# DelphinusLab/halo2-gpu-specific

Hardware: AMD Instinct MI355X
Metric: NTT Fr-ops/s @ k=24 (forward+inverse 2^24 BN254 Fr NTT; MSM G1-adds/s under 'msm') (higher is better)
Workload: dtype u32x8 (254-bit Montgomery, integer)

## Files before the change

halo2-gpu-specific_amd/csrc/field.hpp:

```cpp
#pragma once
#ifdef __HIPCC_RTC__
typedef unsigned char uint8_t;
typedef unsigned short uint16_t;
typedef unsigned int uint32_t;
typedef unsigned long uint64_t;
typedef int int32_t;
typedef long int64_t;
#else
#include <hip/hip_runtime.h>
#include <stdint.h>
#endif

namespace h2 {

struct FrParams {
    static constexpr uint32_t MOD[8] = {0xf0000001u, 0x43e1f593u, 0x79b97091u, 0x2833e848u,
                                        0x8181585du, 0xb85045b6u, 0xe131a029u, 0x30644e72u};
    static constexpr uint32_t MOD2[8] = {0xe0000002u, 0x87c3eb27u, 0xf372e122u, 0x5067d090u,
                                         0x0302b0bau, 0x70a08b6du, 0xc2634053u, 0x60c89ce5u};
    static constexpr uint32_t MOD4[8] = {0xc0000004u, 0x0f87d64fu, 0xe6e5c245u, 0xa0cfa121u,
                                         0x06056174u, 0xe14116dau, 0x84c680a6u, 0xc19139cbu};
    static constexpr uint32_t NMOD[8] = {0x0fffffffu, 0xbc1e0a6cu, 0x86468f6eu, 0xd7cc17b7u,
                                         0x7e7ea7a2u, 0x47afba49u, 0x1ece5fd6u, 0xcf9bb18du};
    static constexpr uint32_t PINV256[8] = {0xefffffffu, 0xc2e1f593u, 0x4c6911b3u, 0x6586864bu,
// ... 348 lines not shown
    d.l[1] = subb_co(a.l[1], b.l[1], ca);
    u.l[0] = add_co(d.l[0], P::MOD2[0], cb);
#pragma unroll
    for (int i = 2; i < 8; i++) {
        d.l[i] = subb_co(a.l[i], b.l[i], ca);
        u.l[i - 1] = addc_co(d.l[i - 1], P::MOD2[i - 1], cb);
    }
    u.l[7] = addc_co(d.l[7], P::MOD2[7], cb);
#pragma unroll
    for (int i = 0; i < 8; i++) r.l[i] = sel_co(d.l[i], u.l[i], ca);
    return r;
#else
    return fp_lazy_red2p(fp_lazy_sub(a, b));
#endif
}
template <class P>
H2_DEV Fp<P> fp_lazy_canon(const Fp<P>& a) {
    return fp_reduce_once(fp_lazy_red2p(a));
}

template <int CL>
struct alignas(16) FpChunk {
    uint32_t w[64 / CL];
};

H2_DEV void mad_acc(uint64_t& lo, uint32_t& hi, uint32_t a, uint32_t b) {
#if defined(H2_PORTABLE_MUL) || !defined(__HIP_DEVICE_COMPILE__)
    uint64_t p = (uint64_t)a * b;
    uint64_t s = lo + p;
    hi += (s < p) ? 1u : 0u;
    lo = s;
#else
    uint64_t carry;
    asm("v_mad_u64_u32 %0, %1, %2, %3, %0" : "+v"(lo), "=s"(carry) : "v"(a), "v"(b));
    asm("v_addc_co_u32 %0, %1, %0, 0, %1" : "+v"(hi), "+s"(carry));
#endif
}

template <class P>
__device__ __forceinline__ Fp<P> fp_mul_dev(const Fp<P>& a, const Fp<P>& b);
template <class P>
__device__ __forceinline__ Fp<P> fp_sqr_dev(const Fp<P>& a);
template <class P>
__device__ __forceinline__ Fp<P> fp_mul2_dev(const Fp<P>& a, const Fp<P>& b, const Fp<P>& c, const Fp<P>& d);
template <class P>
__device__ __forceinline__ Fp<P> fp_mul_wide_dev(const Fp<P>& a, const Fp<P>& b);
template <class P>
__device__ __forceinline__ Fp<P> fp_mul_const_dev(const Fp<P>& a, const Fp<P>& w, const Fp<P>& wq);
template <class P, int CL>
__device__ __forceinline__ Fp<P> fp_mul_chunk_dev(const Fp<P>& a, const FpChunk<CL>& t);
#if defined(__HIP_DEVICE_COMPILE__) && !defined(H2_PORTABLE_MUL)
#include "fp_mul_gen.hpp"
#endif

template <class P>
H2_DEV Fp<P> fp_mul(const Fp<P>& a, const Fp<P>& b) {
#if !defined(__HIP_DEVICE_COMPILE__)
    {
        typedef unsigned __int128 u128;
        uint64_t x[4], y[4], p[4];
        for (int i = 0; i < 4; i++) {
            x[i] = (uint64_t)a.l[2 * i] | ((uint64_t)a.l[2 * i + 1] << 32);
            y[i] = (uint64_t)b.l[2 * i] | ((uint64_t)b.l[2 * i + 1] << 32);
            p[i] = (uint64_t)P::MOD[2 * i] | ((uint64_t)P::MOD[2 * i + 1] << 32);
        }
        uint64_t inv = p[0];
        for (int i = 0; i < 6; i++) inv *= 2 - p[0] * inv;
        inv = 0 - inv;
        uint64_t t[6] = {0, 0, 0, 0, 0, 0};
        for (int i = 0; i < 4; i++) {
            u128 c = 0;
            for (int j = 0; j < 4; j++) {
                c += (u128)t[j] + (u128)x[j] * y[i];
                t[j] = (uint64_t)c;
                c >>= 64;
            }
            c += t[4];
            t[4] = (uint64_t)c;
            t[5] = (uint64_t)(c >> 64);
            const uint64_t m = t[0] * inv;
            c = ((u128)t[0] + (u128)m * p[0]) >> 64;
            for (int j = 1; j < 4; j++) {
                c += (u128)t[j] + (u128)m * p[j];
                t[j - 1] = (uint64_t)c;
                c >>= 64;
            }
            c += t[4];
            t[3] = (uint64_t)c;
            t[4] = t[5] + (uint64_t)(c >> 64);
        }
        Fp<P> r;
        for (int i = 0; i < 4; i++) {
            r.l[2 * i] = (uint32_t)t[i];
            r.l[2 * i + 1] = (uint32_t)(t[i] >> 32);
        }
        return fp_reduce_once(r);
    }
#elif !defined(H2_PORTABLE_MUL)
    return fp_mul_dev(a, b);
#endif
    Fp<P> r;
    uint64_t lo = 0;
    uint32_t hi = 0;
    uint32_t m[8];
#pragma unroll
    for (int i = 0; i < 8; i++) {
#pragma unroll
        for (int j = 0; j <= i; j++) mad_acc(lo, hi, a.l[j], b.l[i - j]);
#pragma unroll
        for (int j = 0; j < i; j++) mad_acc(lo, hi, m[j], P::MOD[i - j]);
        m[i] = (uint32_t)lo * P::INV;
        mad_acc(lo, hi, m[i], P::MOD[0]);
        lo = (lo >> 32) | ((uint64_t)hi << 32);
        hi = 0;
    }
#pragma unroll
    for (int i = 8; i < 16; i++) {
#pragma unroll
        for (int j = i - 7; j < 8; j++) mad_acc(lo, hi, a.l[j], b.l[i - j]);
#pragma unroll
        for (int j = i - 7; j < 8; j++) mad_acc(lo, hi, m[j], P::MOD[i - j]);
        r.l[i - 8] = (uint32_t)lo;
        lo = (lo >> 32) | ((uint64_t)hi << 32);
        hi = 0;
    }
    return fp_reduce_once(r);
}

template <class P>
H2_DEV Fp<P> fp_sqr(const Fp<P>& a) {
#if defined(__HIP_DEVICE_COMPILE__) && !defined(H2_PORTABLE_MUL) && !defined(H2_NO_SQR)
    return fp_sqr_dev(a);
#else
    return fp_mul(a, a);
#endif
}

template <class P>
H2_DEV Fp<P> fp_mul2(const Fp<P>& a, const Fp<P>& b, const Fp<P>& c, const Fp<P>& d) {
#if defined(__HIP_DEVICE_COMPILE__) && !defined(H2_PORTABLE_MUL) && !defined(H2_NO_MUL2)
    return fp_mul2_dev(a, b, c, d);
#else
    return fp_add(fp_mul(a, b), fp_mul(c, d));
#endif
}

template <class P>
H2_DEV Fp<P> fp_mul_wide(const Fp<P>& a, const Fp<P>& b) {
#if defined(__HIP_DEVICE_COMPILE__) && !defined(H2_PORTABLE_MUL)
    return fp_mul_wide_dev(a, b);
#else
    Fp<P> r;
    uint64_t lo = 0;
    uint32_t hi = 0;
    uint32_t m[8];
    for (int i = 0; i < 8; i++) {
        for (int j = 0; j <= i; j++) mad_acc(lo, hi, a.l[j], b.l[i - j]);
        for (int j = 0; j < i; j++) mad_acc(lo, hi, m[j], P::MOD[i - j]);
        m[i] = (uint32_t)lo * P::INV;
        mad_acc(lo, hi, m[i], P::MOD[0]);
        lo = (lo >> 32) | ((uint64_t)hi << 32);
        hi = 0;
    }
    for (int i = 8; i < 16; i++) {
        for (int j = i - 7; j < 8; j++) mad_acc(lo, hi, a.l[j], b.l[i - j]);
        for (int j = i - 7; j < 8; j++) mad_acc(lo, hi, m[j], P::MOD[i - j]);
        r.l[i - 8] = (uint32_t)lo;
        lo = (lo >> 32) | ((uint64_t)hi << 32);
        hi = 0;
    }
    return r;
#endif
}

template <class P>
H2_DEV Fp<P> fp_mul_const(const Fp<P>& x, const Fp<P>& w, const Fp<P>& wq) {
#if defined(__HIP_DEVICE_COMPILE__) && !defined(H2_PORTABLE_MUL)
    Fp<P> r = fp_mul_const_dev(x, w, wq);
    if (__builtin_expect(r.l[7] >= P::MOD2[7], 0)) r = fp_lazy_red2p(r);
    return r;
#else
    uint32_t q[8];
    {
        uint64_t lo = 0;
        uint32_t hi = 0;
        for (int i = 0; i < 15; i++) {
            for (int j = (i > 7 ? i - 7 : 0); j <= (i < 7 ? i : 7); j++) mad_acc(lo, hi, x.l[j], wq.l[i - j]);
            if (i >= 8) q[i - 8] = (uint32_t)lo;
            lo = (lo >> 32) | ((uint64_t)hi << 32);
            hi = 0;
        }
        q[7] = (uint32_t)lo;
    }
    Fp<P> r;
    uint64_t lo = 0;
    uint32_t hi = 0;
    for (int i = 0; i < 8; i++) {
        for (int j = 0; j <= i; j++) {
            mad_acc(lo, hi, x.l[j], w.l[i - j]);
            mad_acc(lo, hi, q[j], P::NMOD[i - j]);
        }
        r.l[i] = (uint32_t)lo;
        lo = (lo >> 32) | ((uint64_t)hi << 32);
        hi = 0;
    }
    return r;
#endif
}
template <class P>
H2_DEV void fp_const_pair(const Fp<P>& w_mont, Fp<P>& w_plain, Fp<P>& wq) {
    w_plain = fp_from_mont(w_mont);
    uint64_t lo = 0;
    uint32_t hi = 0;
    for (int i = 0; i < 8; i++) {
        for (int j = 0; j <= i; j++) mad_acc(lo, hi, w_mont.l[j], P::PINV256[i - j]);
        wq.l[i] = (uint32_t)lo;
        lo = (lo >> 32) | ((uint64_t)hi << 32);
        hi = 0;
    }
}

template <int CL, class P>
H2_DEV Fp<P> fp_mul_chunk(const Fp<P>& x, const FpChunk<CL>& t) {
#if defined(__HIP_DEVICE_COMPILE__) && !defined(H2_PORTABLE_MUL)
    return fp_mul_chunk_dev<P, CL>(x, t);
#else
    constexpr int NC = 8 / CL, NM = CL + 1;
    Fp<P> r;
    uint64_t lo = 0;
    uint32_t hi = 0;
    uint32_t m[NM];
    for (int i = 0; i < NM + 7; i++) {
        for (int j = 0; j < 8; j++) {
            const int l = i - j % CL;
            if (l >= 0 && l <= 7) mad_acc(lo, hi, x.l[j], t.w[l * NC + j / CL]);
        }
        for (int j = 0; j < NM && j < i; j++)
            if (i - j <= 7) mad_acc(lo, hi, m[j], P::MOD[i - j]);
        if (i < NM) {
            m[i] = (uint32_t)lo * P::INV;
            mad_acc(lo, hi, m[i], P::MOD[0]);
        } else {
            r.l[i - NM] = (uint32_t)lo;
        }
        lo = (lo >> 32) | ((uint64_t)hi << 32);
        hi = 0;
    }
    r.l[7] = (uint32_t)lo;
    return r;
#endif
}
template <int AH, bool SREG = false, class P, class Fetch>
H2_DEV Fp<P> fp_mul_chunk_planes(const Fp<P>& x, Fetch&& fetch) {
#if defined(__HIP_DEVICE_COMPILE__) && !defined(H2_PORTABLE_MUL)
    if constexpr (SREG) return fp_mul_chunk1_splanes_dev<AH>(x, fetch);
    else return fp_mul_chunk1_planes_dev<AH>(x, fetch);
#else
    FpChunk<1> t;
    for (int c = 0; c < 8; c++) {
        uint32_t w[8];
        fetch(w, c);
        for (int k = 0; k < 8; k++) t.w[8 * c + k] = w[k];
    }
    return fp_mul_chunk<1>(x, t);
#endif
}
enum FirstPair { FIRST_PAIR_2P = 0, FIRST_PAIR_4P = 1, FIRST_PAIR_CANON = 2 };
template <class P, class Mul>
H2_DEV void fp_lazy_first_pair_mul(Fp<P>& x0, Fp<P>& x1, Fp<P>& x2, Fp<P>& x3, Mul&& mul, const FirstPair form) {
    Fp<P> y0, y1, y2;
    if (form == FIRST_PAIR_CANON) {
        y0 = fp_lazy_add(x0, x1);
        y1 = fp_lazy_sub_off<1>(x0, x1);
        y2 = fp_lazy_add(x2, x3);
    } else {
        if (form == FIRST_PAIR_4P) {
            x0 = fp_lazy_red2p(x0);
            x1 = fp_lazy_red2p(x1);
            x2 = fp_lazy_red2p(x2);
            x3 = fp_lazy_red2p(x3);
        }
        y0 = fp_lazy_add_red(x0, x1);
        y1 = fp_lazy_sub_red(x0, x1);
        y2 = fp_lazy_red2p(fp_lazy_add(x2, x3));
    }
    const Fp<P> y3 = mul(fp_lazy_sub(x2, x3));
    x0 = fp_lazy_add(y0, y2);
    x1 = fp_lazy_add(y1, y3);
    x2 = fp_lazy_sub(y0, y2);
    x3 = fp_lazy_sub(y1, y3);
}
template <int CL, class P>
H2_DEV void fp_lazy_first_pair_of(Fp<P>& x0, Fp<P>& x1, Fp<P>& x2, Fp<P>& x3, const FpChunk<CL>& w3, const FirstPair form) {
    fp_lazy_first_pair_mul(x0, x1, x2, x3, [&w3](const Fp<P>& d) { return fp_mul_chunk(d, w3); }, form);
}
template <int CL, class P>
H2_DEV void fp_lazy_first_pair(Fp<P>& x0, Fp<P>& x1, Fp<P>& x2, Fp<P>& x3, const FpChunk<CL>& w3, const bool red) {
    fp_lazy_first_pair_of(x0, x1, x2, x3, w3, red ? FIRST_PAIR_4P : FIRST_PAIR_2P);
}
template <int CL, class P>
H2_DEV void fp_lazy_first_pair_canon(Fp<P>& x0, Fp<P>& x1, Fp<P>& x2, Fp<P>& x3, const FpChunk<CL>& w3) {
    fp_lazy_first_pair_of(x0, x1, x2, x3, w3, FIRST_PAIR_CANON);
}
template <int CL, class P>
H2_DEV void fp_chunk_table(const Fp<P>& w_mont, FpChunk<CL>& out) {
    constexpr int NC = 8 / CL;
    const Fp<P> w_plain = fp_from_mont(w_mont);
    for (int k = 0; k < NC; k++) {
        Fp<P> c;
        for (int l = 0; l < 8; l++) c.l[l] = P::CHUNK_POW[CL * k + CL - 1][l];
        const Fp<P> t = fp_mul(w_plain, c);
        for (int l = 0; l < 8; l++) out.w[l * NC + k] = t.l[l];
    }
}

template <class P>
H2_DEV Fp<P> fp_to_mont(const Fp<P>& canon) {
    Fp<P> rr;
#pragma unroll
    for (int i = 0; i < 8; i++) rr.l[i] = P::RR[i];
    return fp_reduce_once(fp_mul_wide(canon, rr));
}
template <class P>
H2_DEV Fp<P> fp_from_mont(const Fp<P>& a) {
    Fp<P> one = fp_zero<P>();
    one.l[0] = 1;
    return fp_reduce_once(fp_mul_wide(a, one));
}

template <class P>
H2_DEV Fp<P> fp_inv(const Fp<P>& a) {
    uint32_t u[8], v[8], r[8], s[8];
    uint32_t nz = 0;
#pragma unroll
    for (int i = 0; i < 8; i++) {
        u[i] = P::MOD[i];
        v[i] = a.l[i];
        r[i] = 0;
        s[i] = i == 0 ? 1u : 0u;
        nz |= a.l[i];
    }
    if (nz == 0) return a;
    uint32_t k = 0;
    auto halve = [](uint32_t* x) {
#pragma unroll
        for (int i = 0; i < 8; i++) x[i] = (x[i] >> 1) | (i < 7 ? x[i + 1] << 31 : 0u);
    };
    auto dbl = [](uint32_t* x) {
#pragma unroll
        for (int i = 7; i >= 0; i--) x[i] = (x[i] << 1) | (i ? x[i - 1] >> 31 : 0u);
    };
    auto sub = [](uint32_t* x, const uint32_t* y) {
        uint32_t bw = 0;
#pragma unroll
        for (int i = 0; i < 8; i++) {
            const uint32_t d = x[i] - y[i], b1 = x[i] < y[i] ? 1u : 0u, e = d - bw, b2 = d < bw ? 1u : 0u;
            x[i] = e;
            bw = b1 | b2;
        }
    };
    auto add = [](uint32_t* x, const uint32_t* y) {
        uint32_t cy = 0;
#pragma unroll
        for (int i = 0; i < 8; i++) {
            const uint32_t t = x[i] + y[i], c1 = t < y[i] ? 1u : 0u, e = t + cy, c2 = e < cy ? 1u : 0u;
            x[i] = e;
            cy = c1 | c2;
        }
    };
    auto greater = [](const uint32_t* x, const uint32_t* y) {
#pragma unroll
        for (int i = 7; i >= 0; i--)
            if (x[i] != y[i]) return x[i] > y[i];
        return false;
    };
    for (;;) {
        uint32_t vnz = 0;
#pragma unroll
        for (int i = 0; i < 8; i++) vnz |= v[i];
        if (vnz == 0) break;
        if ((u[0] & 1) == 0) {
            halve(u);
            dbl(s);
        } else if ((v[0] & 1) == 0) {
            halve(v);
            dbl(r);
        } else if (greater(u, v)) {
            sub(u, v);
            halve(u);
            add(r, s);
            dbl(s);
        } else {
            sub(v, u);
            halve(v);
            add(s, r);
            dbl(r);
        }
        k++;
    }
    Fp<P> x;
    {
        uint32_t d[8];
        uint64_t bw = 0;
#pragma unroll
        for (int i = 0; i < 8; i++) {
            uint64_t e = (uint64_t)r[i] - P::MOD[i] - bw;
            d[i] = (uint32_t)e;
            bw = (e >> 32) & 1;
        }
        uint64_t bw2 = 0;
#pragma unroll
        for (int i = 0; i < 8; i++) {
            const uint32_t rr = bw ? r[i] : d[i];
            uint64_t e = (uint64_t)P::MOD[i] - rr - bw2;
            x.l[i] = (uint32_t)e;
            bw2 = (e >> 32) & 1;
        }
    }
    x = fp_reduce_once(x);
    for (uint32_t i = k; i < 512; i++) x = fp_dbl(x);
    return x;
}

template <class P>
H2_DEV Fp<P> fp_pow_u32(const Fp<P>& a, uint32_t e) {
    if (e == 0) return fp_one<P>();
    Fp<P> acc = a;
    for (int i = 30 - __builtin_clz(e); i >= 0; i--) {
        acc = fp_sqr(acc);
        if ((e >> i) & 1) acc = fp_mul(acc, a);
    }
    return acc;
}

}
```

halo2-gpu-specific_amd/csrc/ntt_pass.hip:

```cpp
#include <stdexcept>

#include "ntt_pass.hpp"

namespace h2 {

__device__ __forceinline__ void tw_store(Fr* out, uint32_t i, const Fr& w_mont, uint32_t pair) {
    if (!pair) {
        fp_store(out + i, w_mont);
        return;
    }
    if (pair == 2) {
        TwChunk t;
        fp_chunk_table(w_mont, t);
        uint4* const q = reinterpret_cast<uint4*>(out) + (size_t)i * TW_CHUNK_Q;
#pragma unroll
        for (uint32_t k = 0; k < TW_CHUNK_Q; k++) q[k] = make_uint4(t.w[4 * k], t.w[4 * k + 1], t.w[4 * k + 2], t.w[4 * k + 3]);
        return;
    }
    if (pair == 3) {
        TwChunk32 t;
        fp_chunk_table(w_mont, t);
        uint4* const q = reinterpret_cast<uint4*>(out) + (size_t)i * TW_CHUNK32_Q;
#pragma unroll
        for (uint32_t k = 0; k < TW_CHUNK32_Q; k++) q[k] = make_uint4(t.w[4 * k], t.w[4 * k + 1], t.w[4 * k + 2], t.w[4 * k + 3]);
// ... 46 lines not shown
        hi >>= a.prevB[q];
        K |= d << a.prevT[q];
    }
    return K;
}
__device__ __forceinline__ uint32_t K_to_hi(uint32_t K, const PassArgs& a) {
    uint32_t hi = 0;
    for (uint32_t q = 0; q < a.nprev; q++) {
        uint32_t d = (K >> a.prevT[q]) & ((1u << a.prevB[q]) - 1);
        hi = (hi << a.prevB[q]) | d;
    }
    return hi;
}

__device__ __forceinline__ Fr twiddle_pow(const PassArgs& a, uint32_t e) {
    if (a.log_n <= LO_BITS) return fp_load(a.tw_lo + e);
    Fr lo = fp_load(a.tw_lo + (e & ((1u << LO_BITS) - 1)));
    Fr hi = fp_load(a.tw_hi + (e >> LO_BITS));
    return fp_mul(lo, hi);
}

extern __shared__ __attribute__((aligned(16))) uint4 h2_smem[];

__device__ __forceinline__ Fr lds_get(const uint4* lo, const uint4* hi, uint32_t i) {
    uint4 a = lo[i], b = hi[i];
    Fr r;
    r.l[0] = a.x; r.l[1] = a.y; r.l[2] = a.z; r.l[3] = a.w;
    r.l[4] = b.x; r.l[5] = b.y; r.l[6] = b.z; r.l[7] = b.w;
    return r;
}
__device__ __forceinline__ void lds_put(uint4* lo, uint4* hi, uint32_t i, const Fr& v) {
    lo[i] = make_uint4(v.l[0], v.l[1], v.l[2], v.l[3]);
    hi[i] = make_uint4(v.l[4], v.l[5], v.l[6], v.l[7]);
}

__device__ __forceinline__ Fr store_twiddle(const PassArgs& a, const Fr& y, const uint32_t entry) {
    const uint4* const q = reinterpret_cast<const uint4*>(a.nx_tab) + (size_t)entry * TW_CHUNK_Q;
    TwChunk t;
#pragma unroll
    for (uint32_t k = 0; k < TW_CHUNK_Q; k++) {
        const uint4 v = q[k];
        t.w[4 * k] = v.x; t.w[4 * k + 1] = v.y; t.w[4 * k + 2] = v.z; t.w[4 * k + 3] = v.w;
    }
    return fp_mul_chunk(y, t);
}

template <bool RADIX4, bool NLAST = false, bool ST = false>
__global__ void __launch_bounds__(512, 4) k_ntt_pass(PassArgs a) {
    constexpr bool CW = RADIX4;
    static_assert(!ST || NLAST || !RADIX4, "a last pass stores the transform's output");
    const bool is_last = NLAST ? false : a.is_last != 0;
    auto tmul = [](const Fr& x, const Fr& w) -> Fr { return fp_mul_wide(x, w); };
    const uint32_t B = a.B, R = 1u << B, log_c = a.log_c, C = 1u << log_c;
    const uint32_t zskip = a.zskip;
    uint4* t_lo = h2_smem;
    uint4* t_hi = t_lo + (R << log_c);
    uint4* w_lo = t_hi + (R << log_c);
    uint4* w_hi = w_lo + (R >> 1) + (CW ? 0 : 1);
    uint4* q_lo = w_hi + (R >> 1);
    uint4* q_hi = q_lo + (R >> 1);
    struct Tw {
        Fr w, q;
    };
    auto tw_get = [&](uint32_t i) __attribute__((always_inline)) -> Tw {
        Tw t;
        t.w = lds_get(w_lo, w_hi, i);
        if constexpr (CW) t.q = lds_get(q_lo, q_hi, i);
        return t;
    };
    auto bmul = [](const Fr& x, const Tw& t) __attribute__((always_inline)) -> Fr {
        if constexpr (CW) return fp_mul_const(x, t.w, t.q);
        else return fp_mul_wide(x, t.w);
    };
    const uint32_t nthreads = blockDim.x;
    const uint32_t tid = threadIdx.x;
    const Fr* const in_p = a.batch ? a.in_b[blockIdx.y] : a.in;
    Fr* const out_p = a.batch ? a.out_b[blockIdx.y] : a.out;
    const uint32_t n_mask = (a.log_n >= 32) ? 0xffffffffu : ((1u << a.log_n) - 1);

    for (uint32_t i = tid; i < (R >> 1); i += nthreads) {
        if constexpr (CW) {
            lds_put(w_lo, w_hi, i, fp_load(a.tw_bfly + 2 * i));
            lds_put(q_lo, q_hi, i, fp_load(a.tw_bfly + 2 * i + 1));
        } else {
            lds_put(w_lo, w_hi, i, fp_load(a.tw_bfly + i));
        }
    }

    const uint32_t tile_id = blockIdx.x;
    const uint32_t total = R << log_c;

    uint32_t base = 0, K_uniform = 0;
    const uint32_t S = 1u << a.s_log;
    if (!is_last) {
        uint32_t chunks_per_hi = S >> log_c;
        uint32_t hi = tile_id / chunks_per_hi, lo0 = (tile_id % chunks_per_hi) << log_c;
        base = (hi << (B + a.s_log)) + lo0;
        K_uniform = hi_to_K(hi, a);
    }

    constexpr uint32_t NE = RADIX4 ? 4 : 2;
    for (uint32_t e0 = tid; e0 < total; e0 += NE * nthreads) {
        uint32_t rho[NE], col[NE], idx[NE], Kk[NE];
        bool live[NE];
        Fr x[NE];
#pragma unroll
        for (uint32_t q = 0; q < NE; q++) {
            const uint32_t e = e0 + q * nthreads;
            if (!is_last) {
                col[q] = e & (C - 1);
                rho[q] = (e >> log_c) & (R - 1);
                idx[q] = base + (rho[q] << a.s_log) + col[q];
                Kk[q] = K_uniform;
            } else {
                rho[q] = e & (R - 1);
                col[q] = (e >> B) & (C - 1);
                Kk[q] = (tile_id << log_c) + col[q];
                idx[q] = (K_to_hi(Kk[q], a) << B) + rho[q];
            }
            live[q] = e < total && !(zskip && rho[q] >= (R >> zskip));
        }
#pragma unroll
        for (uint32_t q = 0; q < NE; q++) {
            x[q] = fp_zero<FrParams>();
            if (live[q] && idx[q] < a.in_len) x[q] = fp_load(in_p + idx[q]);
        }
        if (a.has_pre3) {
#pragma unroll
            for (uint32_t q = 0; q < NE; q++) {
                const uint32_t m = idx[q] % 3;
                Fr w;
#pragma unroll
                for (int l = 0; l < 8; l++) w.l[l] = m == 1 ? a.pre3[1].l[l] : a.pre3[2].l[l];
                if (m != 0) x[q] = tmul(x[q], w);
            }
        }
        const bool pre_scale = a.scale_mode == 1u && a.nprev == 0;
        if ((a.nprev != 0 && !a.tw_applied) || pre_scale) {
            if (!NLAST && a.tw_direct != nullptr && !pre_scale) {
#pragma unroll
                for (uint32_t q0 = 0; q0 < NE; q0 += 2) {
                    Fr w[2];
#pragma unroll
                    for (uint32_t q = 0; q < 2; q++) w[q] = fp_load(a.tw_direct + ((Kk[q0 + q] << B) | rho[q0 + q]));
#pragma unroll
                    for (uint32_t q = 0; q < 2; q++) x[q0 + q] = tmul(x[q0 + q], w[q]);
                }
            } else if (a.log_n <= LO_BITS && !pre_scale) {
#pragma unroll
                for (uint32_t q = 0; q < NE; q++) {
                    const uint32_t ex = (uint32_t)(((uint64_t)rho[q] * Kk[q]) << a.s_log) & n_mask;
                    x[q] = tmul(x[q], fp_load(a.tw_lo + ex));
                }
            } else {
                const Fr* const two_lo = pre_scale ? a.sc_lo : a.tw_lo;
                const Fr* const two_hi = pre_scale ? a.sc_hi : a.tw_hi;
#pragma unroll
                for (uint32_t q0 = 0; q0 < NE; q0 += 2) {
                    Fr wl[2], wh[2];
#pragma unroll
                    for (uint32_t q = 0; q < 2; q++) {
                        const uint32_t ex = pre_scale ? (idx[q0 + q] & n_mask)
                                                      : ((uint32_t)(((uint64_t)rho[q0 + q] * Kk[q0 + q]) << a.s_log) & n_mask);
                        wl[q] = fp_load(two_lo + (ex & ((1u << LO_BITS) - 1)));
                        wh[q] = fp_load(two_hi + (ex >> LO_BITS));
                    }
#pragma unroll
                    for (uint32_t q = 0; q < 2; q++) x[q0 + q] = tmul(x[q0 + q], fp_mul(wl[q], wh[q]));
                }
            }
        }
#pragma unroll
        for (uint32_t q = 0; q < NE; q++) {
            const uint32_t e = e0 + q * nthreads;
            const uint32_t r_q = is_last ? (e & (R - 1)) : ((e >> log_c) & (R - 1));
            const uint32_t c_q = is_last ? ((e >> B) & (C - 1)) : (e & (C - 1));
            if (e >= total || (zskip && r_q >= (R >> zskip))) continue;
            if (zskip) {
                for (uint32_t m = 0; m < (1u << zskip); m++) lds_put(t_lo, t_hi, ((bitrev(r_q, B) | m) << log_c) + c_q, x[q]);
            } else {
                lds_put(t_lo, t_hi, (bitrev(r_q, B) << log_c) + c_q, x[q]);
            }
        }
    }
    __syncthreads();

    uint32_t s0 = zskip;
    if constexpr (RADIX4) {
        const uint32_t nunits = total >> 2;
        auto round4 = [&](const uint32_t s) __attribute__((always_inline)) {
            const uint32_t h = 1u << s;
            const uint32_t log_per = (B - 2 + log_c) - s;
            const bool by_r = s != 0 && log_per >= 6 && (nthreads & 63) == 0;
            for (uint32_t t = tid; t < nunits; t += nthreads) {
                uint32_t c, r, p;
                if (by_r) {
                    r = t >> log_per;
                    const uint32_t j = t & ((1u << log_per) - 1);
                    c = j & (C - 1);
                    p = ((j >> log_c) << (s + 2)) | r;
                } else {
                    c = t & (C - 1);
                    const uint32_t b = t >> log_c;
                    r = b & (h - 1);
                    p = ((b >> s) << (s + 2)) | r;
                }
                const uint32_t i0 = (p << log_c) + c, step = h << log_c;
                Fr x0 = lds_get(t_lo, t_hi, i0), x1 = lds_get(t_lo, t_hi, i0 + step);
                Fr x2 = lds_get(t_lo, t_hi, i0 + 2 * step), x3 = lds_get(t_lo, t_hi, i0 + 3 * step);
                const bool unit = s == 0 || (by_r && r == 0);
                x0 = fp_lazy_red2p(x0);
                x2 = fp_lazy_red2p(x2);
                if (!unit) {
                    const Tw wa = tw_get(r << (B - 1 - s));
                    x1 = bmul(x1, wa);
                    x3 = bmul(x3, wa);
                } else {
                    x1 = fp_lazy_red2p(x1);
                    x3 = fp_lazy_red2p(x3);
                }
                const Fr y0 = fp_lazy_add_red(x0, x1), y1 = fp_lazy_sub_red(x0, x1);
                Fr y2 = fp_lazy_add(x2, x3), y3 = fp_lazy_sub(x2, x3);
                y2 = unit ? fp_lazy_red2p(y2) : bmul(y2, tw_get(r << (B - 2 - s)));
                y3 = bmul(y3, tw_get((r + h) << (B - 2 - s)));
                lds_put(t_lo, t_hi, i0, fp_lazy_add(y0, y2));
                lds_put(t_lo, t_hi, i0 + 2 * step, fp_lazy_sub(y0, y2));
                lds_put(t_lo, t_hi, i0 + step, fp_lazy_add(y1, y3));
                lds_put(t_lo, t_hi, i0 + 3 * step, fp_lazy_sub(y1, y3));
            }
            __syncthreads();
        };
        for (; s0 + 1 < B; s0 += 2) round4(s0);
    }
    const uint32_t nbf = total >> 1;
    for (uint32_t s = s0; s < B; s++) {
        const uint32_t h = 1u << s;
        const uint32_t log_per = (B - 1 + log_c) - s;
        const bool by_r = s != 0 && log_per >= 6 && (nthreads & 63) == 0;
        for (uint32_t t = tid; t < nbf; t += nthreads) {
            uint32_t c, r, i;
            if (by_r) {
                r = t >> log_per;
                uint32_t j = t & ((1u << log_per) - 1);
                c = j & (C - 1);
                i = ((j >> log_c) << (s + 1)) | r;
            } else {
                c = t & (C - 1);
                uint32_t b = t >> log_c;
                r = b & (h - 1);
                i = ((b >> s) << (s + 1)) | r;
            }
            const uint32_t iu = (i << log_c) + c, iv = ((i + h) << log_c) + c;
            Fr u = lds_get(t_lo, t_hi, iu), v = lds_get(t_lo, t_hi, iv);
            const bool skip = s == 0 || (by_r && r == 0);
            u = fp_lazy_red2p(u);
            v = skip ? fp_lazy_red2p(v) : bmul(v, tw_get(r << (B - 1 - s)));
            lds_put(t_lo, t_hi, iu, fp_lazy_add(u, v));
            lds_put(t_lo, t_hi, iv, fp_lazy_sub(u, v));
        }
        __syncthreads();
    }

    for (uint32_t e0 = tid; e0 < total; e0 += NE * nthreads) {
        Fr y[NE];
        uint32_t idx[NE];
#pragma unroll
        for (uint32_t q = 0; q < NE; q++) {
            const uint32_t e = e0 + q * nthreads;
            const uint32_t c = e & (C - 1), k = (e >> log_c) & (R - 1);
            if (!is_last)
                idx[q] = base + (k << a.s_log) + c;
            else
                idx[q] = ((tile_id << log_c) + c) + (k << a.t_log);
            y[q] = lds_get(t_lo, t_hi, (k << log_c) + c);
        }
        if (is_last && a.scale_mode == 2u) {
#pragma unroll
            for (uint32_t q = 0; q < NE; q++) {
                const uint32_t i = idx[q] & n_mask;
                const Fr w = fp_mul(fp_load(a.sc_lo + (i & ((1u << LO_BITS) - 1))), fp_load(a.sc_hi + (i >> LO_BITS)));
                y[q] = fp_reduce_once(fp_mul_wide(y[q], w));
            }
        } else if (is_last && a.has_post3 && !a.hi_scaled) {
#pragma unroll
            for (uint32_t q = 0; q < NE; q++) {
                const uint32_t m = idx[q] % 3;
                Fr w;
#pragma unroll
                for (int l = 0; l < 8; l++) w.l[l] = m == 0 ? a.post3[0].l[l] : (m == 1 ? a.post3[1].l[l] : a.post3[2].l[l]);
                y[q] = fp_reduce_once(fp_mul_wide(y[q], w));
            }
        } else if (is_last) {
#pragma unroll
            for (uint32_t q = 0; q < NE; q++) y[q] = fp_lazy_canon(y[q]);
        }
        if constexpr (ST) {
#pragma unroll
            for (uint32_t q = 0; q < NE; q++) {
                const uint32_t e = e0 + q * nthreads;
                const uint32_t rho_n = (idx[q] >> a.nx_s_log) & ((1u << a.nx_B) - 1);
                const uint32_t K_n = K_uniform | (((e >> log_c) & (R - 1)) << a.t_log);
                if (e < total) y[q] = store_twiddle(a, y[q], (rho_n << a.nx_t_log) | K_n);
            }
        }
#pragma unroll
        for (uint32_t q = 0; q < NE; q++)
            if (e0 + q * nthreads < total) fp_store(out_p + idx[q], y[q]);
    }
}

static constexpr uint32_t PASS8_TW_LDS = 32;
static constexpr uint32_t PASS8_LDS = ((256u << 2) * 2 + PASS8_TW_LDS * TW_CHUNK_Q) * sizeof(uint4);
static_assert(4 * PASS8_LDS <= 160u * 1024, "four workgroups of k_ntt_pass8 per CU");
template <bool NLAST, bool ST = false>
__global__ void __launch_bounds__(256, 4) k_ntt_pass8(PassArgs a) {
    static_assert(!ST || NLAST, "a last pass stores the transform's output");
    constexpr uint32_t B = 8, R = 1u << B, log_c = 2, C = 1u << log_c;
    auto tmul = [](const Fr& x, const Fr& w) -> Fr { return fp_mul_wide(x, w); };
    uint4* t_lo = h2_smem;
    uint4* t_hi = t_lo + (R << log_c);
    uint4* w_pl = t_hi + (R << log_c);
    const uint4* const tw_tab = reinterpret_cast<const uint4*>(a.tw_chunk);
    using Tw = TwChunk;
    auto tw_unpack = [](Tw& t, const uint32_t k, const uint4 v) __attribute__((always_inline)) {
        t.w[4 * k] = v.x; t.w[4 * k + 1] = v.y; t.w[4 * k + 2] = v.z; t.w[4 * k + 3] = v.w;
    };
    static_assert((R >> 1) / PASS8_TW_LDS == 4, "the stage pairs before the last read the indices that are multiples of 4");
    auto tw_get = [&](const uint32_t i, const bool mem) __attribute__((always_inline)) -> Tw {
        Tw t;
#pragma unroll
        for (uint32_t k = 0; k < TW_CHUNK_Q; k++)
            tw_unpack(t, k, mem ? tw_tab[(size_t)i * TW_CHUNK_Q + k] : w_pl[k * PASS8_TW_LDS + (i >> 2)]);
        return t;
    };
    auto bmul = [](const Fr& x, const Tw& t) __attribute__((always_inline)) -> Fr { return fp_mul_chunk(x, t); };
    typedef const __attribute__((address_space(4))) uint32_t* TwScalar;
    const TwScalar tw32_s = (TwScalar)reinterpret_cast<const uint32_t*>(a.tw_chunk32);
    auto bmul_s = [&](const Fr& x, const uint32_t i) __attribute__((always_inline)) -> Fr {
        const TwScalar e = tw32_s + (i >> 2) * (uint32_t)(sizeof(TwChunk32) / sizeof(uint32_t));
        return fp_mul_chunk_planes<1, true>(x, [e](uint32_t (&w)[8], const uint32_t c) __attribute__((always_inline)) {
#pragma unroll
            for (uint32_t k = 0; k < 8; k++) w[k] = e[8 * c + k];
        });
    };
    auto unit4_mul = [&](Fr& x0, Fr& x1, Fr& x2, Fr& x3, const uint32_t s, const uint32_t r, const bool unit) __attribute__((always_inline)) {
        const uint32_t h = 1u << s;
        const bool mem = s == B - 2;
        const bool uni = s == 2;
        x0 = fp_lazy_red2p(x0);
        Fr y2, n3;
        if (!unit) {
            if (uni) {
                x1 = bmul_s(x1, r << (B - 1 - s));
                x3 = bmul_s(x3, r << (B - 1 - s));
            } else {
                const Tw wa = tw_get(r << (B - 1 - s), mem);
                x1 = bmul(x1, wa);
                x3 = bmul(x3, wa);
            }
            y2 = fp_lazy_add(x2, x3);
            n3 = fp_lazy_sub_from4p(x3, x2);
        } else {
            x1 = fp_lazy_red2p(x1);
            x2 = fp_lazy_red2p(x2);
            x3 = fp_lazy_red2p(x3);
            y2 = fp_lazy_add(x2, x3);
            n3 = fp_lazy_sub(x3, x2);
        }
        const Fr y0 = fp_lazy_add_red(x0, x1), y1 = fp_lazy_sub_red(x0, x1);
        if (uni) {
            y2 = unit ? fp_lazy_red2p(y2) : bmul_s(y2, r << (B - 2 - s));
            n3 = bmul_s(n3, (r + h) << (B - 2 - s));
        } else {
            y2 = unit ? fp_lazy_red2p(y2) : bmul(y2, tw_get(r << (B - 2 - s), mem));
            n3 = bmul(n3, tw_get((r + h) << (B - 2 - s), mem));
        }
        x0 = y0;
        x1 = y1;
        x2 = y2;
        x3 = n3;
    };
    auto unit4_add = [](Fr& x0, Fr& x1, Fr& x2, Fr& x3) __attribute__((always_inline)) {
        const Fr y0 = x0, y1 = x1, y2 = x2, n3 = x3;
        x0 = fp_lazy_add(y0, y2);
        x1 = fp_lazy_sub(y1, n3);
        x2 = fp_lazy_sub(y0, y2);
        x3 = fp_lazy_add(y1, n3);
    };
    auto unit_of = [](const uint32_t tid, const uint32_t s, uint32_t& i0, uint32_t& r, bool& unit) __attribute__((always_inline)) {
        const uint32_t h = 1u << s, log_per = (B - 2 + log_c) - s;
        const bool by_r = s != 0 && log_per >= 6;
        uint32_t c, p;
        if (by_r) {
            r = tid >> log_per;
            const uint32_t j = tid & ((1u << log_per) - 1);
            c = j & (C - 1);
            p = ((j >> log_c) << (s + 2)) | r;
        } else {
            c = tid & (C - 1);
            const uint32_t b = tid >> log_c;
            r = b & (h - 1);
            p = ((b >> s) << (s + 2)) | r;
        }
        i0 = (p << log_c) + c;
        unit = s == 0 || (by_r && r == 0);
    };
    const uint32_t tid = threadIdx.x;
    const uint32_t wave = __builtin_amdgcn_readfirstlane(tid >> 6);
    auto round4 = [&](const uint32_t s) __attribute__((always_inline)) {
        uint32_t i0, r;
        bool unit;
        unit_of(tid, s, i0, r, unit);
        if (s == 2) {
            r = wave;
            unit = wave == 0;
        }
        const uint32_t step = (1u << s) << log_c;
        Fr x0 = lds_get(t_lo, t_hi, i0), x1 = lds_get(t_lo, t_hi, i0 + step);
        Fr x2 = lds_get(t_lo, t_hi, i0 + 2 * step), x3 = lds_get(t_lo, t_hi, i0 + 3 * step);
        unit4_mul(x0, x1, x2, x3, s, r, unit);
        unit4_add(x0, x1, x2, x3);
        lds_put(t_lo, t_hi, i0, x0);
        lds_put(t_lo, t_hi, i0 + 2 * step, x2);
        lds_put(t_lo, t_hi, i0 + step, x1);
        lds_put(t_lo, t_hi, i0 + 3 * step, x3);
        __syncthreads();
    };
    const bool is_last = NLAST ? false : a.is_last != 0;
    const uint32_t n_mask = (a.log_n >= 32) ? 0xffffffffu : ((1u << a.log_n) - 1);

    static_assert(PASS8_TW_LDS * TW_CHUNK_Q == 256, "one word of the LDS copy per lane");
    const uint4 w_fill = tw_tab[(size_t)(tid / TW_CHUNK_Q) * 4 * TW_CHUNK_Q + tid % TW_CHUNK_Q];


    constexpr uint32_t NE = 4;
    {
        const uint32_t tile_id = blockIdx.x;
        const Fr* const in_p = a.batch ? a.in_b[blockIdx.y] : a.in;
        Fr* const out_p = a.batch ? a.out_b[blockIdx.y] : a.out;
        uint32_t base = 0, K_uniform = 0;
        if (!is_last) {
            const uint32_t chunks_per_hi = (1u << a.s_log) >> log_c;
            const uint32_t hi = tile_id / chunks_per_hi, lo0 = (tile_id % chunks_per_hi) << log_c;
            base = (hi << (B + a.s_log)) + lo0;
            K_uniform = hi_to_K(hi, a);
        }

        {
            uint32_t rho[NE], col[NE], idx[NE], Kk[NE];
            Fr x[NE];
#pragma unroll
            for (uint32_t q = 0; q < NE; q++) {
                if (!is_last) {
                    col[q] = tid & (C - 1);
                    rho[q] = bitrev(tid >> log_c, B - 2) + (q << (B - 2));
                    idx[q] = base + (rho[q] << a.s_log) + col[q];
                    Kk[q] = K_uniform;
                } else {
                    rho[q] = (tid & 63) + (q << (B - 2));
                    col[q] = tid >> 6;
                    Kk[q] = (tile_id << log_c) + col[q];
                    idx[q] = (K_to_hi(Kk[q], a) << B) + rho[q];
                }
            }
#pragma unroll
            for (uint32_t q = 0; q < NE; q++) {
                x[q] = fp_zero<FrParams>();
                if (idx[q] < a.in_len) x[q] = fp_load(in_p + idx[q]);
            }
            const bool pre_scale = a.scale_mode == 1u && a.nprev == 0;
            const bool direct = !NLAST && a.nprev != 0 && !a.tw_applied && a.tw_direct != nullptr && !pre_scale;
            Fr wd[2];
            if (direct) {
#pragma unroll
                for (uint32_t q = 0; q < 2; q++) wd[q] = fp_load(a.tw_direct + ((Kk[q] << B) | rho[q]));
            }
            __builtin_amdgcn_sched_barrier(0);
            w_pl[(tid % TW_CHUNK_Q) * PASS8_TW_LDS + tid / TW_CHUNK_Q] = w_fill;
            if (a.has_pre3) {
#pragma unroll
                for (uint32_t q = 0; q < NE; q++) {
                    const uint32_t m = idx[q] % 3;
                    Fr w;
#pragma unroll
                    for (int l = 0; l < 8; l++) w.l[l] = m == 1 ? a.pre3[1].l[l] : a.pre3[2].l[l];
                    if (m != 0) x[q] = tmul(x[q], w);
                }
            }
            if ((a.nprev != 0 && !a.tw_applied) || pre_scale) {
                if (direct) {
                    Fr w[2];
#pragma unroll
                    for (uint32_t q = 0; q < 2; q++) w[q] = fp_load(a.tw_direct + ((Kk[2 + q] << B) | rho[2 + q]));
#pragma unroll
                    for (uint32_t q = 0; q < 2; q++) x[q] = tmul(x[q], wd[q]);
#pragma unroll
                    for (uint32_t q = 0; q < 2; q++) x[2 + q] = tmul(x[2 + q], w[q]);
                } else if (a.log_n <= LO_BITS && !pre_scale) {
#pragma unroll
                    for (uint32_t q = 0; q < NE; q++) {
                        const uint32_t ex = (uint32_t)(((uint64_t)rho[q] * Kk[q]) << a.s_log) & n_mask;
                        x[q] = tmul(x[q], fp_load(a.tw_lo + ex));
                    }
                } else {
                    const Fr* const two_lo = pre_scale ? a.sc_lo : a.tw_lo;
                    const Fr* const two_hi = pre_scale ? a.sc_hi : a.tw_hi;
#pragma unroll
                    for (uint32_t q0 = 0; q0 < NE; q0 += 2) {
                        Fr wl[2], wh[2];
#pragma unroll
                        for (uint32_t q = 0; q < 2; q++) {
                            const uint32_t ex = pre_scale ? (idx[q0 + q] & n_mask)
                                                          : ((uint32_t)(((uint64_t)rho[q0 + q] * Kk[q0 + q]) << a.s_log) & n_mask);
                            wl[q] = fp_load(two_lo + (ex & ((1u << LO_BITS) - 1)));
                            wh[q] = fp_load(two_hi + (ex >> LO_BITS));
                        }
#pragma unroll
                        for (uint32_t q = 0; q < 2; q++) x[q0 + q] = tmul(x[q0 + q], fp_mul(wl[q], wh[q]));
                    }
                }
            }
            const uint32_t b = is_last ? bitrev(tid & 63, B - 2) : (tid >> log_c);
            const uint32_t i0 = (b << (2 + log_c)) + (is_last ? (tid >> 6) : (tid & (C - 1)));
            const FirstPair form = (a.nprev != 0 || pre_scale) ? FIRST_PAIR_2P : (a.has_pre3 ? FIRST_PAIR_4P : FIRST_PAIR_CANON);
            fp_lazy_first_pair_mul(x[0], x[2], x[1], x[3], [&](const Fr& d) __attribute__((always_inline)) { return bmul_s(d, R >> 2); }, form);
            lds_put(t_lo, t_hi, i0, x[0]);
            lds_put(t_lo, t_hi, i0 + 2 * C, x[1]);
            lds_put(t_lo, t_hi, i0 + C, x[2]);
            lds_put(t_lo, t_hi, i0 + 3 * C, x[3]);
        }
        __syncthreads();
        round4(2);
        round4(4);

        Fr y[NE];
        const uint4* nx_q = nullptr;
        size_t nx_step = 0;
        if constexpr (ST) {
            const uint32_t rho_n = (base >> a.nx_s_log) & ((1u << a.nx_B) - 1);
            const uint32_t K_n = K_uniform | ((tid >> log_c) << a.t_log);
            nx_q = reinterpret_cast<const uint4*>(a.nx_tab) + (size_t)((rho_n << a.nx_t_log) | K_n) * TW_CHUNK_Q;
            nx_step = (size_t)((R / NE) << a.t_log) * TW_CHUNK_Q;
        }
        Tw nx_t;
        {
            uint32_t i0, r;
            bool unit;
            unit_of(tid, 6, i0, r, unit);
#pragma unroll
            for (uint32_t q = 0; q < NE; q++) y[q] = lds_get(t_lo, t_hi, i0 + q * (R << log_c) / NE);
            unit4_mul(y[0], y[1], y[2], y[3], 6, r, unit);
            if constexpr (ST) {
#pragma unroll
                for (uint32_t k = 0; k < TW_CHUNK_Q; k++) tw_unpack(nx_t, k, nx_q[k]);
                __builtin_amdgcn_sched_barrier(0);
            }
            unit4_add(y[0], y[1], y[2], y[3]);
        }
        uint32_t idx[NE];
#pragma unroll
        for (uint32_t q = 0; q < NE; q++) {
            const uint32_t c = tid & (C - 1), k = (tid >> log_c) + q * (R / NE);
            if (!is_last)
                idx[q] = base + (k << a.s_log) + c;
            else
                idx[q] = ((tile_id << log_c) + c) + (k << a.t_log);
        }
        if (is_last && a.scale_mode == 2u) {
#pragma unroll
            for (uint32_t q = 0; q < NE; q++) {
                const uint32_t i = idx[q] & n_mask;
                const Fr w = fp_mul(fp_load(a.sc_lo + (i & ((1u << LO_BITS) - 1))), fp_load(a.sc_hi + (i >> LO_BITS)));
                y[q] = fp_reduce_once(fp_mul_wide(y[q], w));
            }
        } else if (is_last && a.has_post3 && !a.hi_scaled) {
#pragma unroll
            for (uint32_t q = 0; q < NE; q++) {
                const uint32_t m = idx[q] % 3;
                Fr w;
#pragma unroll
                for (int l = 0; l < 8; l++) w.l[l] = m == 0 ? a.post3[0].l[l] : (m == 1 ? a.post3[1].l[l] : a.post3[2].l[l]);
                y[q] = fp_reduce_once(fp_mul_wide(y[q], w));
            }
        } else if (is_last) {
#pragma unroll
            for (uint32_t q = 0; q < NE; q++) y[q] = fp_lazy_canon(y[q]);
        }
        if constexpr (ST) {
            constexpr uint32_t PF = TW_CHUNK_Q / 2;
#pragma unroll
            for (uint32_t q = 0; q < NE; q++) {
                uint4 pf[PF];
                if (q + 1 < NE) {
#pragma unroll
                    for (uint32_t k = 0; k < PF; k++) pf[k] = nx_q[(q + 1) * nx_step + k];
                    __builtin_amdgcn_sched_barrier(0);
                }
                y[q] = fp_mul_chunk(y[q], nx_t);
                if (q + 1 < NE) {
                    __builtin_amdgcn_sched_barrier(0);
#pragma unroll
                    for (uint32_t k = PF; k < TW_CHUNK_Q; k++) tw_unpack(nx_t, k, nx_q[(q + 1) * nx_step + k]);
#pragma unroll
                    for (uint32_t k = 0; k < PF; k++) tw_unpack(nx_t, k, pf[k]);
                }
            }
        }
#pragma unroll
        for (uint32_t q = 0; q < NE; q++) fp_store(out_p + idx[q], y[q]);
    }
}

using PassFn = void (*)(PassArgs);
static const PassFn pass_fn[H2_NTT_KERNEL_COUNT] = {
    k_ntt_pass8<true>,
    k_ntt_pass8<false>,
    k_ntt_pass<true, true>,
    k_ntt_pass<true, false>,
    k_ntt_pass<false>,
};
static const PassFn pass_fn_st[H2_NTT_KERNEL_COUNT] = {
    k_ntt_pass8<true, true>, nullptr, k_ntt_pass<true, true, true>, nullptr, k_ntt_pass<false, false, true>,
};

void ntt_pass_launch(int device, NttKernel kernel, const PassArgs& a, uint32_t cnt, uint32_t threads, hipStream_t stream) {
    const uint32_t R = 1u << a.B, C = 1u << a.log_c;
    const uint32_t ntiles = (1u << a.log_n) / (R * C);
    const size_t lds = kernel != NK_R2 ? ((size_t)R * C + R) * sizeof(Fr) : ((size_t)R * C + (R >> 1) + 2) * sizeof(Fr);
    if (lds > 64 * 1024) {
        static bool raised[64] = {};
        if (device < 0 || device >= 64 || !raised[device]) {
            for (const PassFn f : {pass_fn[NK_R4_DP], pass_fn[NK_R4], pass_fn[NK_R2], pass_fn_st[NK_R4_DP], pass_fn_st[NK_R2]})
                H2_HIP(hipFuncSetAttribute((const void*)f, hipFuncAttributeMaxDynamicSharedMemorySize, 160 * 1024));
            if (device >= 0 && device < 64) raised[device] = true;
        }
    }
    const bool pass8 = kernel == NK_PASS8_DP || kernel == NK_PASS8;
    const PassFn fn = a.nx_tab ? pass_fn_st[kernel] : pass_fn[kernel];
    if (!fn) throw std::runtime_error("ntt_pass_launch: a last pass has no next pass to multiply for");
    hipLaunchKernelGGL(fn, dim3(ntiles, cnt), dim3(threads), pass8 ? (size_t)PASS8_LDS : lds, stream, a);
}

static dim3 fill_grid(uint32_t count) { return dim3((count + 255) / 256); }

void ntt_fill_pow(Fr* out, const Fr& base, uint32_t mul, uint32_t count, uint32_t form, hipStream_t stream) {
    if (count) hipLaunchKernelGGL(k_pow_table, fill_grid(count), dim3(256), 0, stream, out, base, mul, count, form);
}

void ntt_fill_direct(Fr* out, const Fr& base, uint32_t kbits, uint32_t s_log, uint32_t log_n, uint32_t count, uint32_t form,
                     hipStream_t stream) {
    hipLaunchKernelGGL(k_direct_table, fill_grid(count), dim3(256), 0, stream, out, base, kbits, s_log, log_n, count, form);
}

void ntt_fill_last(Fr* out, const Fr& base, uint32_t bits, uint32_t log_n, const Fr* d, hipStream_t stream) {
    hipLaunchKernelGGL(k_last_table, fill_grid(1u << log_n), dim3(256), 0, stream, out, base, bits, log_n, d ? *d : base,
                       d ? 1u : 0u, 0u);
}

void ntt_fill_scaled(Fr* out, const Fr* in, const Fr& d, uint32_t count, hipStream_t stream) {
    hipLaunchKernelGGL(k_scale_table, fill_grid(count), dim3(256), 0, stream, out, in, d, count);
}

}
```

Before: 472.2 billion.

## Add specialized plain pass8 kernels and loose last-pair butterflies with rare reduction handover

Adds a PLAIN template variant of the radix-256 NTT pass that compiles out batching, bounds-checked loads, pre/post scaling and coset branches. It is dispatched for the common single-transform case as first, middle or last pass. Non-last passes also skip the reducing add/sub in the final butterfly pair and leave outputs loose. A wave-wide ballot then performs a conditional reduction only when some top limb reaches the modulus. The aim is fewer instructions and registers per element, at the cost of more kernel instantiations and looser value bounds that must stay correct across passes.

```diff
diff --git a/halo2-gpu-specific_amd/csrc/field.hpp b/halo2-gpu-specific_amd/csrc/field.hpp
--- a/halo2-gpu-specific_amd/csrc/field.hpp
+++ b/halo2-gpu-specific_amd/csrc/field.hpp
@@ -674,6 +674,37 @@
 H2_DEV void fp_lazy_first_pair_canon(Fp<P>& x0, Fp<P>& x1, Fp<P>& x2, Fp<P>& x3, const FpChunk<CL>& w3) {
     fp_lazy_first_pair_of(x0, x1, x2, x3, w3, FIRST_PAIR_CANON);
 }
+template <class P>
+H2_DEV void fp_lazy_last_pair_loose_head(const Fp<P>& x0, const Fp<P>& x1, Fp<P>& y0, Fp<P>& y1) {
+    y0 = fp_lazy_add(x0, x1);
+    y1 = fp_lazy_sub(x0, x1);
+}
+template <class P>
+H2_DEV void fp_lazy_last_pair_loose_add(Fp<P>& x0, Fp<P>& x1, Fp<P>& x2, Fp<P>& x3) {
+    const Fp<P> y0 = x0, y1 = x1, y2 = x2, n3 = x3;
+    x0 = fp_lazy_add(y0, y2);
+    x1 = fp_lazy_sub_off<1>(y1, n3);
+    x2 = fp_lazy_sub(y0, y2);
+    x3 = fp_lazy_add(y1, n3);
+}
+template <bool BRANCH = true, int N, class P>
+H2_DEV void fp_chunk_handover(Fp<P> (&y)[N]) {
+    bool rare = true;
+    if (BRANCH) {
+        uint32_t top = y[0].l[7];
+#pragma unroll
+        for (int q = 1; q < N; q++) top = y[q].l[7] > top ? y[q].l[7] : top;
+#if defined(__HIP_DEVICE_COMPILE__) && !defined(H2_PORTABLE_MUL)
+        rare = __builtin_expect(__builtin_amdgcn_ballot_w64(top >= P::MOD[7]) != 0, 0);
+#else
+        rare = top >= P::MOD[7];
+#endif
+    }
+    if (rare) {
+#pragma unroll
+        for (int q = 0; q < N; q++) y[q] = fp_reduce_once(y[q]);
+    }
+}
 template <int CL, class P>
 H2_DEV void fp_chunk_table(const Fp<P>& w_mont, FpChunk<CL>& out) {
     constexpr int NC = 8 / CL;
diff --git a/halo2-gpu-specific_amd/csrc/ntt_pass.hip b/halo2-gpu-specific_amd/csrc/ntt_pass.hip
--- a/halo2-gpu-specific_amd/csrc/ntt_pass.hip
+++ b/halo2-gpu-specific_amd/csrc/ntt_pass.hip
@@ -372,6 +372,7 @@
                 const uint32_t K_n = K_uniform | (((e >> log_c) & (R - 1)) << a.t_log);
                 if (e < total) y[q] = store_twiddle(a, y[q], (rho_n << a.nx_t_log) | K_n);
             }
+            fp_chunk_handover<RADIX4>(y);
         }
 #pragma unroll
         for (uint32_t q = 0; q < NE; q++)
@@ -382,7 +383,7 @@
 static constexpr uint32_t PASS8_TW_LDS = 32;
 static constexpr uint32_t PASS8_LDS = ((256u << 2) * 2 + PASS8_TW_LDS * TW_CHUNK_Q) * sizeof(uint4);
 static_assert(4 * PASS8_LDS <= 160u * 1024, "four workgroups of k_ntt_pass8 per CU");
-template <bool NLAST, bool ST = false>
+template <bool NLAST, bool ST = false, bool PLAIN = false>
 __global__ void __launch_bounds__(256, 4) k_ntt_pass8(PassArgs a) {
     static_assert(!ST || NLAST, "a last pass stores the transform's output");
     constexpr uint32_t B = 8, R = 1u << B, log_c = 2, C = 1u << log_c;
@@ -437,7 +438,13 @@
             y2 = fp_lazy_add(x2, x3);
             n3 = fp_lazy_sub(x3, x2);
         }
-        const Fr y0 = fp_lazy_add_red(x0, x1), y1 = fp_lazy_sub_red(x0, x1);
+        Fr y0, y1;
+        if (NLAST && mem) {
+            fp_lazy_last_pair_loose_head(x0, x1, y0, y1);
+        } else {
+            y0 = fp_lazy_add_red(x0, x1);
+            y1 = fp_lazy_sub_red(x0, x1);
+        }
         if (uni) {
             y2 = unit ? fp_lazy_red2p(y2) : bmul_s(y2, r << (B - 2 - s));
             n3 = bmul_s(n3, (r + h) << (B - 2 - s));
@@ -450,7 +457,11 @@
         x2 = y2;
         x3 = n3;
     };
-    auto unit4_add = [](Fr& x0, Fr& x1, Fr& x2, Fr& x3) __attribute__((always_inline)) {
+    auto unit4_add = [](Fr& x0, Fr& x1, Fr& x2, Fr& x3, const bool loose) __attribute__((always_inline)) {
+        if (loose) {
+            fp_lazy_last_pair_loose_add(x0, x1, x2, x3);
+            return;
+        }
         const Fr y0 = x0, y1 = x1, y2 = x2, n3 = x3;
         x0 = fp_lazy_add(y0, y2);
         x1 = fp_lazy_sub(y1, n3);
@@ -489,14 +500,14 @@
         Fr x0 = lds_get(t_lo, t_hi, i0), x1 = lds_get(t_lo, t_hi, i0 + step);
         Fr x2 = lds_get(t_lo, t_hi, i0 + 2 * step), x3 = lds_get(t_lo, t_hi, i0 + 3 * step);
         unit4_mul(x0, x1, x2, x3, s, r, unit);
-        unit4_add(x0, x1, x2, x3);
+        unit4_add(x0, x1, x2, x3, false);
         lds_put(t_lo, t_hi, i0, x0);
         lds_put(t_lo, t_hi, i0 + 2 * step, x2);
         lds_put(t_lo, t_hi, i0 + step, x1);
         lds_put(t_lo, t_hi, i0 + 3 * step, x3);
         __syncthreads();
     };
-    const bool is_last = NLAST ? false : a.is_last != 0;
+    const bool is_last = NLAST ? false : (PLAIN || a.is_last != 0);
     const uint32_t n_mask = (a.log_n >= 32) ? 0xffffffffu : ((1u << a.log_n) - 1);
 
     static_assert(PASS8_TW_LDS * TW_CHUNK_Q == 256, "one word of the LDS copy per lane");
@@ -506,14 +517,14 @@
     constexpr uint32_t NE = 4;
     {
         const uint32_t tile_id = blockIdx.x;
-        const Fr* const in_p = a.batch ? a.in_b[blockIdx.y] : a.in;
-        Fr* const out_p = a.batch ? a.out_b[blockIdx.y] : a.out;
+        const Fr* const in_p = !PLAIN && a.batch ? a.in_b[blockIdx.y] : a.in;
+        Fr* const out_p = !PLAIN && a.batch ? a.out_b[blockIdx.y] : a.out;
         uint32_t base = 0, K_uniform = 0;
         if (!is_last) {
             const uint32_t chunks_per_hi = (1u << a.s_log) >> log_c;
             const uint32_t hi = tile_id / chunks_per_hi, lo0 = (tile_id % chunks_per_hi) << log_c;
             base = (hi << (B + a.s_log)) + lo0;
-            K_uniform = hi_to_K(hi, a);
+            if (!(PLAIN && ST)) K_uniform = hi_to_K(hi, a);
         }
 
         {
@@ -535,11 +546,16 @@
             }
 #pragma unroll
             for (uint32_t q = 0; q < NE; q++) {
-                x[q] = fp_zero<FrParams>();
-                if (idx[q] < a.in_len) x[q] = fp_load(in_p + idx[q]);
-            }
-            const bool pre_scale = a.scale_mode == 1u && a.nprev == 0;
-            const bool direct = !NLAST && a.nprev != 0 && !a.tw_applied && a.tw_direct != nullptr && !pre_scale;
+                if constexpr (PLAIN) {
+                    x[q] = fp_load(in_p + idx[q]);
+                } else {
+                    x[q] = fp_zero<FrParams>();
+                    if (idx[q] < a.in_len) x[q] = fp_load(in_p + idx[q]);
+                }
+            }
+            const bool pre_scale = !PLAIN && a.scale_mode == 1u && a.nprev == 0;
+            const bool direct = PLAIN ? !NLAST : (!NLAST && a.nprev != 0 && !a.tw_applied && a.tw_direct != nullptr && !pre_scale);
+            const bool load_mul = PLAIN ? !NLAST : ((a.nprev != 0 && !a.tw_applied) || pre_scale);
             Fr wd[2];
             if (direct) {
 #pragma unroll
@@ -547,7 +563,7 @@
             }
             __builtin_amdgcn_sched_barrier(0);
             w_pl[(tid % TW_CHUNK_Q) * PASS8_TW_LDS + tid / TW_CHUNK_Q] = w_fill;
-            if (a.has_pre3) {
+            if (!PLAIN && a.has_pre3) {
 #pragma unroll
                 for (uint32_t q = 0; q < NE; q++) {
                     const uint32_t m = idx[q] % 3;
@@ -557,7 +573,7 @@
                     if (m != 0) x[q] = tmul(x[q], w);
                 }
             }
-            if ((a.nprev != 0 && !a.tw_applied) || pre_scale) {
+            if (load_mul) {
                 if (direct) {
                     Fr w[2];
 #pragma unroll
@@ -592,7 +608,9 @@
             }
             const uint32_t b = is_last ? bitrev(tid & 63, B - 2) : (tid >> log_c);
             const uint32_t i0 = (b << (2 + log_c)) + (is_last ? (tid >> 6) : (tid & (C - 1)));
-            const FirstPair form = (a.nprev != 0 || pre_scale) ? FIRST_PAIR_2P : (a.has_pre3 ? FIRST_PAIR_4P : FIRST_PAIR_CANON);
+            const FirstPair form = PLAIN ? (NLAST ? FIRST_PAIR_CANON : FIRST_PAIR_2P)
+                                   : a.tw_applied ? FIRST_PAIR_CANON
+                                   : (a.nprev != 0 || pre_scale) ? FIRST_PAIR_2P : (a.has_pre3 ? FIRST_PAIR_4P : FIRST_PAIR_CANON);
             fp_lazy_first_pair_mul(x[0], x[2], x[1], x[3], [&](const Fr& d) __attribute__((always_inline)) { return bmul_s(d, R >> 2); }, form);
             lds_put(t_lo, t_hi, i0, x[0]);
             lds_put(t_lo, t_hi, i0 + 2 * C, x[1]);
@@ -625,7 +643,7 @@
                 for (uint32_t k = 0; k < TW_CHUNK_Q; k++) tw_unpack(nx_t, k, nx_q[k]);
                 __builtin_amdgcn_sched_barrier(0);
             }
-            unit4_add(y[0], y[1], y[2], y[3]);
+            unit4_add(y[0], y[1], y[2], y[3], NLAST);
         }
         uint32_t idx[NE];
 #pragma unroll
@@ -636,14 +654,14 @@
             else
                 idx[q] = ((tile_id << log_c) + c) + (k << a.t_log);
         }
-        if (is_last && a.scale_mode == 2u) {
+        if (!PLAIN && is_last && a.scale_mode == 2u) {
 #pragma unroll
             for (uint32_t q = 0; q < NE; q++) {
                 const uint32_t i = idx[q] & n_mask;
                 const Fr w = fp_mul(fp_load(a.sc_lo + (i & ((1u << LO_BITS) - 1))), fp_load(a.sc_hi + (i >> LO_BITS)));
                 y[q] = fp_reduce_once(fp_mul_wide(y[q], w));
             }
-        } else if (is_last && a.has_post3 && !a.hi_scaled) {
+        } else if (!PLAIN && is_last && a.has_post3 && !a.hi_scaled) {
 #pragma unroll
             for (uint32_t q = 0; q < NE; q++) {
                 const uint32_t m = idx[q] % 3;
@@ -675,6 +693,11 @@
                     for (uint32_t k = 0; k < PF; k++) tw_unpack(nx_t, k, pf[k]);
                 }
             }
+            fp_chunk_handover(y);
+            uint32_t t = (wave << 6) | __builtin_amdgcn_mbcnt_hi(~0u, __builtin_amdgcn_mbcnt_lo(~0u, 0u));
+            asm volatile("" : "+v"(t) : "v"(y[NE - 1].l[7]));
+#pragma unroll
+            for (uint32_t q = 0; q < NE; q++) idx[q] = base + (((t >> log_c) + q * (R / NE)) << a.s_log) + (t & (C - 1));
         }
 #pragma unroll
         for (uint32_t q = 0; q < NE; q++) fp_store(out_p + idx[q], y[q]);
@@ -693,6 +716,19 @@
     k_ntt_pass8<true, true>, nullptr, k_ntt_pass<true, true, true>, nullptr, k_ntt_pass<false, false, true>,
 };
 
+static const PassFn pass8_plain_first = k_ntt_pass8<true, true, true>, pass8_plain_middle = k_ntt_pass8<true, false, true>,
+                    pass8_plain_last = k_ntt_pass8<false, false, true>;
+static PassFn pass8_plain(NttKernel kernel, const PassArgs& a, uint32_t cnt) {
+    if (cnt != 1 || a.batch || a.in_len < (1u << a.log_n) || a.has_pre3 || a.scale_mode != 0) return nullptr;
+    if (kernel == NK_PASS8) {
+        const bool table = a.nprev != 0 && !a.tw_applied && a.tw_direct != nullptr;
+        return a.is_last && table && !(a.has_post3 && !a.hi_scaled) ? pass8_plain_last : nullptr;
+    }
+    if (kernel != NK_PASS8_DP || a.is_last) return nullptr;
+    if (a.nx_tab) return a.nprev == 0 ? pass8_plain_first : nullptr;
+    return a.nprev != 0 && a.tw_applied ? pass8_plain_middle : nullptr;
+}
+
 void ntt_pass_launch(int device, NttKernel kernel, const PassArgs& a, uint32_t cnt, uint32_t threads, hipStream_t stream) {
     const uint32_t R = 1u << a.B, C = 1u << a.log_c;
     const uint32_t ntiles = (1u << a.log_n) / (R * C);
@@ -706,7 +742,8 @@
         }
     }
     const bool pass8 = kernel == NK_PASS8_DP || kernel == NK_PASS8;
-    const PassFn fn = a.nx_tab ? pass_fn_st[kernel] : pass_fn[kernel];
+    PassFn fn = a.nx_tab ? pass_fn_st[kernel] : pass_fn[kernel];
+    if (const PassFn plain = pass8_plain(kernel, a, cnt)) fn = plain;
     if (!fn) throw std::runtime_error("ntt_pass_launch: a last pass has no next pass to multiply for");
     hipLaunchKernelGGL(fn, dim3(ntiles, cnt), dim3(threads), pass8 ? (size_t)PASS8_LDS : lds, stream, a);
 }
```

Measured after the change: 477.7 billion (median of 6 runs). +1.2%, better.
